# hmchuong/MaGGIe

Hardware: AMD Instinct MI355X
Metric: instance-frames/sec (fwd+bwd+optimizer step, 512x512, bf16) (higher is better)
Workload: dtype bf16

## Files before the change

include/maggie_hip.h:

```cpp
#ifndef MAGGIE_HIP_H
#define MAGGIE_HIP_H
#include <stdint.h>
#ifdef __cplusplus
extern "C" {
#endif

#define MG_F32 0
#define MG_BF16 1
#define MG_F16 3

#define MG_ACT_NONE 0
#define MG_ACT_RELU 1
#define MG_ACT_LRELU 2

#define MG_STAT_REPLICAS 32

#define MG_MODE_CONV 0
#define MG_MODE_TCONV 1
#define MG_MODE_GATHER 2

int mg_abi_version(void);
int mg_set_zeroed_range(void* base, long bytes);
int mg_zero_claim(void* p, long bytes);
int mg_zeroed_range_conflicts(void);

#define MG_DET_STAT_ROWS 1024
int mg_set_deterministic(int on);
int mg_get_deterministic(void);
int mg_det_init(long bytes);
int mg_det_side_stream(void* stream, long bytes);
int mg_stat_rows(void);
int mg_det_reduce_test(const float* slots, int nblk, int groups, int nv, float* dst, void* stream);

typedef struct mg_conv_params {
    const void* x;
    const void* w;
    void* y;
    const int32_t* nbr;
    const float* scale;
    const float* shift;
    const void* res;
    const void* res2;
    float* stats;
    int32_t dtype, mode;
    int32_t N, Hin, Win, Cin, Hout, Wout, Cout, R, S, stride, pad, dil;
    int32_t M;
    int32_t ldx, ldy, yoff, ldr, ldr2;
    int32_t act, pre_act, res_mode;
    float slope;
    int32_t dw_dtype;
    int32_t stat_mode;
    const int32_t* m_dev;
    const void* bnb_y;
    const void* bnb_x;
    const float* bnb_mean;
    const float* bnb_invstd;
    int32_t bnb_act, bnb_ld;
    int32_t stat_rep;
    int32_t reserved0;
    const float* xf_scale;
    const float* xf_shift;
    int32_t xf_act;
    float xf_slope;
    const float* bnb_scale;
    const float* bnb_shift;
} mg_conv_params;

int mg_conv_xform_ok(const mg_conv_params* p, int which);

int mg_conv_fprop(const mg_conv_params* p, void* stream);
int mg_set_halo3(int on);
int mg_set_halo3_cfg(int th, int bn, int ns);
int mg_conv_stat_rows(int M, int N, int Hout, int Wout);
int mg_coop_error(int* out);
int mg_set_bn_coop(int on);
int mg_set_bn_bwd_tail(int on);
long mg_conv_fprop_workspace(const mg_conv_params* p);
int mg_conv_fprop_ws(const mg_conv_params* p, float* workspace, long workspace_floats, void* stream);

int mg_conv_wgrad(const mg_conv_params* p, void* stream);
long mg_conv_wgrad_workspace(const mg_conv_params* p);
int mg_conv_wgrad_ws(const mg_conv_params* p, float* workspace, long workspace_floats, void* stream);
typedef struct mg_wgrad_parked {
    const float* ws;
    void* dw;
    long n;
    int32_t splits, form, dw_dtype, blocks;
} mg_wgrad_parked;
int mg_conv_wgrad_park(const mg_conv_params* p, float* workspace, long workspace_floats, mg_wgrad_parked* out, void* stream);
int mg_wgrad_reduce_batched(const mg_wgrad_parked* items, int count, void* stream);


typedef struct mg_rowwise_params {
    const void* x;
    void* y;
    const void* dy;
    void* dx;
    const void* res;
    const void* res2;
    void* dres;
    const float* scale;
    const float* shift;
    const float* mean;
    const float* invstd;
    float* sums;
    const float* count_ptr;
    int32_t dtype, M, C, H, W;
    int32_t ldx, ldy, yoff, ldr, ldr2, lddy, lddx, lddres;
    int32_t act, res_mode, mask_x_pos;
    float slope, count;
    const int32_t* m_dev;
    int32_t count_mult;
    int32_t mask_from_x;
} mg_rowwise_params;

int mg_colstats(const void* x, int dtype, int M, int C, int ld, float* stats, void* stream);
int mg_colstats_centered(const void* x, int dtype, int M, int C, int ld, float* stats, int have_sum, void* stream);
int mg_stat_rows_sum(const float* stats, int nrep, int n, float* out, void* stream);
int mg_bn_finalize(const float* stats, int nrep, const float* count_ptr, float count, int C, int centered, const float* gamma, const float* beta,
                   float* running_mean, float* running_var, float momentum, float eps, float* scale, float* shift,
                   float* mean_out, float* invstd_out, void* stream);
int mg_bn_train_fwd(const mg_rowwise_params* p, float* stats_ws, int ws_zeroed, float* outs, const float* stats_in, int stats_in_rows,
                    int exact, const float* gamma, const float* beta, float* running_mean, float* running_var, float momentum, float eps,
                    void* stream);
int mg_bn_train_bwd(const mg_rowwise_params* p, int sums_zeroed, void* stream);
int mg_bn_fold(int C, const float* gamma, const float* beta, const float* running_mean, const float* running_var,
               float eps, float* scale, float* shift, void* stream);
int mg_affine_act(const mg_rowwise_params* p, void* stream);
int mg_bn_bwd_reduce(const mg_rowwise_params* p, void* stream);
int mg_bn_bwd_apply(const mg_rowwise_params* p, void* stream);
int mg_bn_bwd_apply_linked(const mg_rowwise_params* p, const float* sums_rep, int nrep, float* sums_out, void* stream);
int mg_pool2x2(const void* in, void* out, int dtype, int op, int N, int Ho, int Wo, int C, void* stream);

#define MG_U8 2
int mg_bits_pack(const void* a, int dtype, void* bits, int P, int H, int W, int mode, float lo, float hi, void* stream);
int mg_bits_unpack_u8(const void* bits, uint8_t* out, int P, int H, int W, void* stream);
int mg_bits_unpack_f32(const void* bits, float* out, int P, int H, int W, void* stream);
int mg_bits_select(const void* bits, const float* a, const float* b, float* out, int P, int H, int W, void* stream);
int mg_bits_select_bwd(const void* bits, const float* dy, float* da, float* db, int P, int H, int W, void* stream);
int mg_bits_dilate(const void* in, void* out, const void* andmask, int P, int H, int W, const int32_t* widths, int width_all,
                   void* stream);
int mg_bits_downsample(const void* fine, void* coarse, int P, int Hf, int Wf, void* stream);
int mg_bits_rank(const void* bits, int P, int H, int W, int32_t* counts_tmp, int32_t* rowoff, int32_t* wordoff, void* stream);
int mg_bits_truncate(void* bits, const int32_t* wordoff, int P, int H, int W, int cap, int32_t* count, int32_t* overflow, void* stream);
int mg_bits_coords(const void* bits, const int32_t* wordoff, int P, int H, int W, int32_t* coords, void* stream);
int mg_gather_table(const int32_t* coords, int R, int ksize, int kind, const void* src_bits, const int32_t* src_wordoff, int Hs,
                    int Ws, int32_t* nbr, void* stream);

int mg_gather_rows(const void* dense, int dtype, const int32_t* coords, int R, int n_i, int Hd, int Wd, int C, const float* mul,
                   int mul_ninst, void* out, int ldo, int yoff, void* stream);
int mg_gather_rows_bwd(const void* dout, int dtype, int ldo, int yoff, const int32_t* coords, int R, int n_i, int Hd, int Wd, int C,
                       const float* mul, int mul_ninst, const void* dense, float* ddense, float* dmul, void* stream);
int mg_gather_rows_dmul_det(const void* dout, int dtype, int ldo, int yoff, const int32_t* coords, int R, int n_i, int N, int Hd, int Wd, int C,
                            int mul_ninst, const void* dense, float* dmul, const int32_t* r_dev, void* stream);
int mg_gather_rows_bwd_dense(const void* dout, int dtype, int ldo, int yoff, const void* bits, const int32_t* wordoff, int n_i, int N,
                             int Hd, int Wd, int C, const float* mul, int mul_ninst, void* ddense, void* stream);
int mg_scatter_plane(const void* vals, int dtype, int ldv, int col, const int32_t* coords, int R, int P, int H, int W, float fill,
                     float* plane, void* stream);
int mg_gather_plane(const float* plane, const int32_t* coords, int R, int H, int W, void* vals, int dtype, int ldv, int col,
                    void* stream);
int mg_mask_embed(const float* image, const float* masks, const float* table, int N, int H, int W, int n_m, int Hm, int Wm,
                  int n_embed, void* out, int dtype, void* stream);
int mg_mask_embed_bwd(const void* dx, int dtype, const float* masks, int N, int H, int W, int n_m, int Hm, int Wm, int n_embed,
                      float* dtable, void* stream);
int mg_upsample_tanh(const void* in, int dtype, long sn, long sc, long sy, long sx, int N, int C, int h, int w, int scale,
                     int apply_tanh, float* out, void* stream);
int mg_upsample_tanh_bwd(const float* dout, const float* out, long sn, long sc, long sy, long sx, int N, int C, int h, int w,
                         int scale, int apply_tanh, float* din, void* stream);
int mg_upsample_tanh_ex(const void* in, int dtype, long sn, long sc, long sy, long sx, int N, int C, int h, int w, int scale,
                        int apply_tanh, float* out, const float* pscale, int32_t* any_nonzero, void* stream);
int mg_upsample_tanh_bwd_ex(const float* dout, const float* out, long sn, long sc, long sy, long sx, int N, int C, int h, int w,
                            int scale, int apply_tanh, float* din, const float* pscale, void* stream);

int mg_spectral_norm(const float* W, float* u, float* v, int A, int B, int taps, int transposed, int pad_in, void* out,
                     int out_dtype, float* work, void* stream);
int mg_spectral_norm_bwd(const float* G, const float* W, const float* u, const float* v, int A, int B, int taps, int transposed,
                         int pad_in, float* work, float* dW, void* stream);

int mg_attn_tok_fwd(const float* qk, const float* btab, const float* feat, const int32_t* ids, int B, int T, int L, int D, int NID,
                    float scale, float* p, float* ctx, void* stream);
int mg_attn_tok_bwd(const float* p, const float* feat, const float* qk, const int32_t* ids, const float* dctx, const float* dp, int B, int T,
                    int L, int D, int NID, float scale, float* gbuf, float* rowdot, float* dqk, float* dbtab, float* dfeat, void* stream);
int mg_attn_feat_fwd(const float* feat, const float* kq, const float* b2, const float* vp, const float* obias, const uint8_t* pad_mask,
                     const int32_t* ids, int B, int T, int L, int D, int NID, float scale, float* out, float* p, void* stream);
int mg_attn_feat_bwd(const float* dout, const float* p, const float* feat, const float* kq, const float* vp, const int32_t* ids, int B, int T,
                     int L, int D, int NID, float scale, float* dfeat, float* dkq, float* dvp, float* db2, float* dobias, void* stream);
int mg_attn_feat_fwd_ex(const float* feat, const float* kq, const float* b2, const float* vp, const float* obias, const uint8_t* pad_mask,
                        const int32_t* ids, int B, int T, int L, int Dm, int NID, float scale, float* out, float* p, int b2_tn, void* stream);
int mg_attn_feat_bwd_ex(const float* dout, const float* p, const float* feat, const float* kq, const float* vp, const int32_t* ids, int B, int T,
                        int L, int Dm, int NID, float scale, float* dfeat, float* dkq, float* dvp, float* db2, float* dobias, int b2_tn, void* stream);

int mg_plane_flags(const float* w, int P, int HW, int32_t* flags, void* stream);
int mg_plane_flags_ex(const float* w, int P, int HW, void* flags, int as_float, void* stream);
int mg_os8_weight(const float* gt, const float* a8, int P, long HW, int reweight, int32_t* flags_scratch, float* out, void* stream);
int mg_os8_weight_ex(const float* gt, const float* a8, int P, long HW, int reweight, int32_t* flags_scratch, float* out, const int32_t* pvalid,
                     void* stream);
int mg_loss_finish(const float* sums, float* out3, void* stream);
int mg_loss_coef(const float* g3, const float* sums, float* coef5, void* stream);
int mg_loss_point_fwd(const float* p, const float* t, const float* w, const int32_t* flags, int P, int H, int W, float* d,
                      float* sums, const int32_t* pvalid, void* stream);
int mg_pyr_down(const float* x, const int32_t* flags, int P, int h, int w, float* out, void* stream);
int mg_pyr_lap_fwd(const float* x, const float* down, const float* w0, int lvl, int H0, int W0, const int32_t* flags, int P, int h,
                   int w, float* G, float* sums, void* stream);
int mg_pyr_upT(const float* q, const float* coef, const float* add, const int32_t* flags, int P, int h, int w, float* r, void* stream);
int mg_pyr_downT(const float* r, const float* q, const float* coef, const int32_t* flags, int P, int h, int w, float* dd, void* stream);
int mg_loss_point_bwd(const float* p, const float* t, const float* w, const int32_t* flags, int P, int H, int W, const float* coef_rec,
                      const float* coef_grad, const float* dd, float* A, float* B, float* dp, const int32_t* pvalid, void* stream);

int mg_matting_losses_fwd(const float* const* p, const float* t, const float* const* w, const int32_t* pvalid, int S, int P, int H, int W, int32_t* flags,
                          float* d, float* down0, float* down1, float* down2, float* G0, float* G1, float* G2, float* sums, float* out, void* stream);
int mg_matting_losses_bwd(const float* g, const float* sums, const float* const* p, const float* t, const float* const* w, const int32_t* pvalid,
                          const int32_t* flags, int S, int P, int H, int W, const float* G0, const float* G1, const float* G2, float* coef, float* r2,
                          float* dd2, float* r1, float* dd1, float* r0, float* dd0, float* A, float* B, float* dp, void* stream);

typedef struct mg_sn_desc {
    const float* W;
    float* u;
    float* v;
    int64_t out_off;
    int64_t work_off;
    int64_t dw_off;
    int32_t A, B, taps, transposed, pad_in;
    int32_t plain;
    int32_t k3_first, k3_count;
} mg_sn_desc;
// ... 153 lines not shown
```

maggie_amd/csrc/conv_wgrad.hip:

```cpp
#include "common.h"
#include "conv_xcd.h"
#include "../../include/maggie_hip.h"
#include <stdlib.h>
#include <type_traits>

#define MG_STAMP(i)

namespace {

typedef __attribute__((ext_vector_type(4))) short s16x4;
typedef s16x4 __attribute__((address_space(3))) * lds_s16x4_ptr;

template <typename T, int TCO, int TCI, int MODE, bool XF = false>
__global__ __launch_bounds__(256) void igemm_wgrad_kernel(const mg_conv_params p, int rows_per_block, float* __restrict__ ws) {
    using TR = ElemTraits<T>;
    constexpr int CE = TR::CE;
    constexpr bool BF = sizeof(T) == 2;
    constexpr int KSTEP = BF ? 128 : 64;
    constexpr int WROWS = KSTEP / 4;
    constexpr int PAD = BF ? 8 : 16;
    constexpr int PCO = TCO + PAD, PCI = TCI + PAD;
    constexpr int CPY = TCO / CE, CPX = TCI / CE;
    constexpr int ITY = (KSTEP * CPY) / 256, ITX = (KSTEP * CPX) / 256;
    constexpr int FM = TCO / 16, FN = TCI / 16;
    static_assert((KSTEP * CPY) % 256 == 0 && (KSTEP * CPX) % 256 == 0, "tile/threads mismatch");

    extern __shared__ __attribute__((aligned(16))) char smem[];
    T* sY = (T*)smem;
    T* sX = (T*)(smem + KSTEP * PCO * sizeof(T));

    const int t = threadIdx.x, lane = t & 63, wave = t >> 6;
    const int li = lane & 15, g = lane >> 4;
    const int taps = p.R * p.S;
    const int nci = (p.Cin + TCI - 1) / TCI;
    const int nco = (p.Cout + TCO - 1) / TCO;
    int nsplit = (p.M + rows_per_block - 1) / rows_per_block;
    const int M = dev_rows(p.m_dev, p.M);
    if (p.m_dev) {
        rows_per_block = (((M + nsplit - 1) / nsplit + KSTEP - 1) / KSTEP) * KSTEP;
        if (rows_per_block < KSTEP) rows_per_block = KSTEP;
    }
    int work;
    if (!xcd_order(nsplit * taps * nci * nco, work)) return;
    const int tc = work % (taps * nci);
    const int rest = work / (taps * nci);
    const int split = rest / nco;
    const int tap = tc / nci;
    const int ci0 = (tc - tap * nci) * TCI;
    const int co0 = (rest - split * nco) * TCO;
    const int mbeg = split * rows_per_block;
    const int mend = min(M, mbeg + rows_per_block);
    if (mbeg >= mend && !p.m_dev) return;
    const int ky = tap / p.S, kx = tap - ky * p.S;
    const FastDiv div_hw(MODE == MG_MODE_GATHER ? 1 : p.Hout * p.Wout), div_w(MODE == MG_MODE_GATHER ? 1 : p.Wout);
    const int sshift = p.stride == 1 ? 0 : (p.stride == 2 ? 1 : (p.stride == 4 ? 2 : -1));
    const T* __restrict__ yb = (const T*)p.y;
    const T* __restrict__ xb = (const T*)p.x;
    const bool yvec = (p.ldy % CE == 0) && (p.yoff % CE == 0);

    uint4 ry[ITY], rx[ITX];
    [[maybe_unused]] float xsc[CE < 8 ? 8 : CE], xsh[CE < 8 ? 8 : CE];
    [[maybe_unused]] unsigned xlive = 0;
    [[maybe_unused]] const float xsl = xf_slope_of(p.xf_act, p.xf_slope);
    if constexpr (XF) {
        static_assert(BF && 256 % CPX == 0, "operand transform: 16-bit storage, one channel group per thread");
        const int c = t % CPX;
#pragma unroll
        for (int e = 0; e < 8; ++e) {
            const int ci = ci0 + c * CE + e;
            xsc[e] = ci < p.Cin ? p.xf_scale[ci] : 0.f; xsh[e] = ci < p.Cin ? p.xf_shift[ci] : 0.f;
        }
    }
    auto load_step = [&](int mb) {
#pragma unroll
        for (int i = 0; i < ITY; ++i) {
            int idx = t + i * 256;
            int row = idx / CPY, c = idx - row * CPY;
            int m = mb + row, co = co0 + c * CE;
            uint4 q = make_uint4(0, 0, 0, 0);
            if (m < mend && co < p.Cout) {
                const T* src = yb + (long)m * p.ldy + p.yoff + co;
                if (yvec && co + CE <= p.Cout) q = *(const uint4*)src;
                else {
                    float f[CE];
#pragma unroll
                    for (int e = 0; e < CE; ++e) f[e] = (co + e < p.Cout) ? TR::ld(src + e) : 0.f;
                    q = TR::pack(f);
                }
            }
            ry[i] = q;
        }
#pragma unroll
        for (int i = 0; i < ITX; ++i) {
            int idx = t + i * 256;
            int row = idx / CPX, c = idx - row * CPX;
            int m = mb + row, ci = ci0 + c * CE;
            long src = -1;
            if (m < mend && ci < p.Cin) {
                if (MODE == MG_MODE_GATHER) {
                    src = p.nbr[(long)m * taps + tap];
                } else {
                    int n, rem, ho, wo;
                    div_hw.divmod(m, n, rem);
                    div_w.divmod(rem, ho, wo);
                    if (MODE == MG_MODE_CONV) {
                        int hi = ho * p.stride - p.pad + ky * p.dil, wi = wo * p.stride - p.pad + kx * p.dil;
                        if (hi >= 0 && hi < p.Hin && wi >= 0 && wi < p.Win) src = ((long)n * p.Hin + hi) * p.Win + wi;
                    } else {
                        int th = ho + p.pad - ky * p.dil, tw = wo + p.pad - kx * p.dil;
                        if (th >= 0 && tw >= 0) {
                            int hi, wi;
                            if (sshift >= 0) { hi = th >> sshift; wi = tw >> sshift; }
                            else { hi = th / p.stride; wi = tw / p.stride; }
                            if (hi * p.stride == th && wi * p.stride == tw && hi < p.Hin && wi < p.Win)
                                src = ((long)n * p.Hin + hi) * p.Win + wi;
                        }
                    }
                }
            }
            rx[i] = (src >= 0) ? *(const uint4*)(xb + src * p.ldx + ci) : make_uint4(0, 0, 0, 0);
            if constexpr (XF) xlive = src >= 0 ? (xlive | (1u << i)) : (xlive & ~(1u << i));
        }
    };
    auto store_step = [&]() {
#pragma unroll
        for (int i = 0; i < ITY; ++i) {
            int idx = t + i * 256; int row = idx / CPY, c = idx - row * CPY;
            *(uint4*)(sY + row * PCO + c * CE) = ry[i];
        }
#pragma unroll
        for (int i = 0; i < ITX; ++i) {
            int idx = t + i * 256; int row = idx / CPX, c = idx - row * CPX;
            if constexpr (XF) { if (xlive & (1u << i)) rx[i] = xf_apply8<T>(rx[i], xsc, xsh, xsl); }
            *(uint4*)(sX + row * PCI + c * CE) = rx[i];
        }
    };

    f32x4 acc[FM][FN];
#pragma unroll
    for (int i = 0; i < FM; ++i)
#pragma unroll
        for (int j = 0; j < FN; ++j) acc[i][j] = (f32x4){0.f, 0.f, 0.f, 0.f};

    const int wr = wave * WROWS;
    load_step(mbeg);
    for (int mb = mbeg; mb < mend; mb += KSTEP) {
        store_step();
        __syncthreads();
        if (mb + KSTEP < mend) load_step(mb + KSTEP);
        if constexpr (BF) {
            s16x4 a[FM][2], b[FN][2];
            const int r0 = wr + g * 4 + (li >> 2), cq = (li & 3) * 4;
#pragma unroll
            for (int i = 0; i < FM; ++i) {
                a[i][0] = __builtin_amdgcn_ds_read_tr16_b64_v4i16((lds_s16x4_ptr)(sY + r0 * PCO + i * 16 + cq));
                a[i][1] = __builtin_amdgcn_ds_read_tr16_b64_v4i16((lds_s16x4_ptr)(sY + (r0 + 16) * PCO + i * 16 + cq));
            }
#pragma unroll
            for (int j = 0; j < FN; ++j) {
// ... 495 lines not shown
    constexpr int ITY = NY / 256;
    extern __shared__ __attribute__((aligned(16))) char smem[];
    bf16raw* sY = (bf16raw*)smem;
    bf16raw* sX = sY + TH * TW * PY;

    const int t = threadIdx.x, lane = t & 63, wave = t >> 6;
    const int li = lane & 15, g = lane >> 4;
    const int mt = wave & 1, pair = wave >> 1;
    const int nco = p.Cout / TCO;
    const int tiles_x = (p.Wout + TW - 1) / TW, tiles_y = (p.Hout + TH - 1) / TH;
    const int S = p.N * tiles_y * tiles_x;
    const int nsplit = (S + tiles_per_block - 1) / tiles_per_block;
    int work;
    if (!xcd_order(nsplit * nco, work)) return;
    const int co0 = (work % nco) * TCO, split = work / nco;
    const int s_beg = split * tiles_per_block, s_end = min(S, s_beg + tiles_per_block);
    const bf16raw* __restrict__ yb = (const bf16raw*)p.y;
    const bf16raw* __restrict__ xb = (const bf16raw*)p.x;

    int y_ty[ITY], y_tx[ITY], y_off[ITY];
#pragma unroll
    for (int i = 0; i < ITY; ++i) {
        const int idx = t + i * 256;
        const int px = idx >> 2, c = idx & 3;
        y_ty[i] = px / TW; y_tx[i] = px % TW;
        y_off[i] = (y_ty[i] * p.Wout + y_tx[i]) * p.ldy + c * 8;
    }
    const int x_hy = t < NX ? t / HW_ - 1 : (1 << 20), x_hx = t % HW_ - 1;
    const int x_off = t < NX ? (x_hy * p.Win + x_hx) * p.ldx : 0;
    if (t < 4) *(uint4*)(sX + (NX + t) * 8) = make_uint4(0, 0, 0, 0);
    uint4 ry[ITY], rx;
    auto load_tile = [&](int s) {
        const int n = s / (tiles_y * tiles_x);
        const int r = s - n * tiles_y * tiles_x;
        const int y0 = (r / tiles_x) * TH, x0 = (r % tiles_x) * TW;
        const bf16raw* ybase = yb + ((long)(n * p.Hout + y0) * p.Wout + x0) * p.ldy + p.yoff + co0;
        const bf16raw* xbase = xb + ((long)(n * p.Hin + y0) * p.Win + x0) * p.ldx;
#pragma unroll
        for (int i = 0; i < ITY; ++i)
            ry[i] = (y0 + y_ty[i] < p.Hout && x0 + y_tx[i] < p.Wout) ? *(const uint4*)(ybase + y_off[i]) : make_uint4(0, 0, 0, 0);
        rx = ((unsigned)(y0 + x_hy) < (unsigned)p.Hin && (unsigned)(x0 + x_hx) < (unsigned)p.Win) ? *(const uint4*)(xbase + x_off) : make_uint4(0, 0, 0, 0);
    };
    auto store_tile = [&]() {
#pragma unroll
        for (int i = 0; i < ITY; ++i) {
            const int idx = t + i * 256;
            *(uint4*)(sY + (idx >> 2) * PY + (idx & 3) * 8) = ry[i];
        }
        if (t < NX) *(uint4*)(sX + t * 8) = rx;
    };

    f32x4 acc[3];
#pragma unroll
    for (int ky = 0; ky < 3; ++ky) acc[ky] = (f32x4){0.f, 0.f, 0.f, 0.f};
    const int q = g * 4 + (li >> 2), cq = (li & 3) * 4;
    if (s_beg < s_end) load_tile(s_beg);
    for (int s = s_beg; s < s_end; ++s) {
        store_tile();
        __syncthreads();
        if (s + 1 < s_end) load_tile(s + 1);
#pragma unroll
        for (int kc = 0; kc < TH / 2; ++kc) {
            union { s16x4 h[2]; uint4 v; } ua, ub;
            ua.h[0] = __builtin_amdgcn_ds_read_tr16_b64_v4i16((lds_s16x4_ptr)(sY + ((2 * kc) * TW + q) * PY + mt * 16 + cq));
            ua.h[1] = __builtin_amdgcn_ds_read_tr16_b64_v4i16((lds_s16x4_ptr)(sY + ((2 * kc + 1) * TW + q) * PY + mt * 16 + cq));
#pragma unroll
            for (int ky = 0; ky < 3; ++ky) {
                ub.h[0] = __builtin_amdgcn_ds_read_tr16_b64_v4i16((lds_s16x4_ptr)(sX + ((2 * kc + ky) * HW_ + q + 2 * pair) * 8 + cq));
                ub.h[1] = __builtin_amdgcn_ds_read_tr16_b64_v4i16((lds_s16x4_ptr)(sX + ((2 * kc + 1 + ky) * HW_ + q + 2 * pair) * 8 + cq));
                acc[ky] = mfma16<T>(ua.v, ub.v, acc[ky]);
            }
        }
        __syncthreads();
    }
    float* __restrict__ slab = ws + (long)split * p.Cout * 72;
    const int kx = 2 * pair + (li >> 3), ci = li & 7;
    if (kx < 3) {
#pragma unroll
        for (int ky = 0; ky < 3; ++ky)
#pragma unroll
            for (int e = 0; e < 4; ++e)
                slab[((long)(co0 + mt * 16 + g * 4 + e) * 9 + ky * 3 + kx) * 8 + ci] = acc[ky][e];
    }
}

static inline bool wgrad_c8_eligible(const mg_conv_params& p) {
    static const int on = [] { const char* e = getenv("MG_WGRAD_C8"); return e ? atoi(e) : 1; }();
    return on && MG_IS16(p.dtype) && p.mode == MG_MODE_CONV && !p.m_dev && p.R == 3 && p.S == 3 && p.stride == 1 && p.pad == 1 && p.dil == 1 &&
           p.Hout == p.Hin && p.Wout == p.Win && p.Cin == 8 && p.Cout % 32 == 0 && p.ldx % 8 == 0 && p.ldy % 8 == 0 && p.yoff % 8 == 0 &&
           p.Wout >= 16 && p.Hout >= 8;
}
static long plan_wgrad_c8(const mg_conv_params& p, int* tpb_out) {
    const long S = (long)p.N * ((p.Hout + 7) / 8) * ((p.Wout + 15) / 16);
    const long nco = p.Cout / 32;
    long splits = (512 + nco - 1) / nco;
    if (splits > S) splits = S;
    if (splits < 1) splits = 1;
    const int tpb = (int)((S + splits - 1) / splits);
    splits = (S + tpb - 1) / tpb;
    if (tpb_out) *tpb_out = tpb;
    return splits;
}
static int launch_wgrad_c8(const mg_conv_params& p, float* ws, long ws_floats, hipStream_t st) {
    int tpb = 1;
    const long splits = plan_wgrad_c8(p, &tpb);
    const long n = (long)p.Cout * 72;
    const bool out_bf16 = MG_IS16(p.dw_dtype);
    if (!ws || ws_floats < splits * n) return -4;
    dim3 grid(xcd_grid(splits * (p.Cout / 32)));
    const size_t lds = (size_t)(8 * 16 * (32 + 16) + (10 * 18 + 4) * 8) * sizeof(bf16raw);
    if (p.dtype == MG_F16) hipLaunchKernelGGL(igemm_wgrad_c8_kernel<f16raw>, grid, dim3(256), lds, st, p, tpb, ws);
    else hipLaunchKernelGGL(igemm_wgrad_c8_kernel<bf16raw>, grid, dim3(256), lds, st, p, tpb, ws);
    const long b = (n + 31) / 32;
    MG_REDUCE_LAUNCH(wgrad_reduce_tile_kernel, b, ws, splits);
    MG_CHECK_LAUNCH();
    return 0;
}

static inline bool wgrad_halo_eligible(const mg_conv_params& p) {
    static const int on = [] { const char* e = getenv("MG_WGRAD_HALO"); return e ? atoi(e) : 1; }();
    return on && MG_IS16(p.dtype) && p.mode == MG_MODE_CONV && !p.m_dev && p.R == 3 && p.S == 3 && p.stride == 1 && p.pad == 1 && p.dil == 1 &&
           p.Hout == p.Hin && p.Wout == p.Win && p.Cin % 32 == 0 && p.Cout % 32 == 0 && p.ldx % 8 == 0 && p.ldy % 8 == 0 && p.yoff % 8 == 0 &&
           p.Wout >= 16 && p.Hout >= 8 && (long)p.Cout * 9 * p.Cin <= (16l << 20);
}

struct WgradHaloPlan { long splits; int tpb; };

static WgradHaloPlan plan_wgrad_halo(const mg_conv_params& p) {
    const long cc = (long)(p.Cin / 32) * (p.Cout / 32);
    const long S = (long)p.N * ((p.Hout + 7) / 8) * ((p.Wout + 15) / 16);
    static const long target = [] { const char* e = getenv("MG_WGRAD_HALO_BLOCKS"); return e ? atol(e) : 256l; }();
    const long n = (long)p.Cout * 9 * p.Cin;
    long splits = (target + cc - 1) / cc;
    if (splits > S) splits = S;
    if (splits > (16l << 20) / n) splits = (16l << 20) / n;
    if (splits < 1) splits = 1;
    const int tpb = (int)((S + splits - 1) / splits);
    splits = (S + tpb - 1) / tpb;
    return {splits, tpb};
}

static int launch_wgrad_halo(const mg_conv_params& p, float* ws, long ws_floats, hipStream_t st) {
    const WgradHaloPlan pl = plan_wgrad_halo(p);
    const long n = (long)p.Cout * 9 * p.Cin;
    const bool out_bf16 = MG_IS16(p.dw_dtype);
    float* use_ws = nullptr;
    if ((pl.splits > 1 || out_bf16) && ws && ws_floats >= pl.splits * n) use_ws = ws;
    if (out_bf16 && !use_ws) return -4;
    if (pl.splits > 1 && !use_ws) return -4;
    if (pl.splits == 1 && !out_bf16) use_ws = p.stats;
    const long cc = (long)(p.Cin / 32) * (p.Cout / 32);
    dim3 grid(xcd_grid(pl.splits * cc));
    const size_t lds = (size_t)(8 * 16 * (32 + 16) + 10 * 18 * (32 + 16)) * sizeof(bf16raw);
    if (p.xf_scale) {
        if (p.dtype == MG_F16) hipLaunchKernelGGL((igemm_wgrad_halo_kernel<1, 1, f16raw, true>), grid, dim3(256), lds, st, p, pl.tpb, use_ws);
        else hipLaunchKernelGGL((igemm_wgrad_halo_kernel<1, 1, bf16raw, true>), grid, dim3(256), lds, st, p, pl.tpb, use_ws);
    } else if (p.dtype == MG_F16) hipLaunchKernelGGL((igemm_wgrad_halo_kernel<1, 1, f16raw>), grid, dim3(256), lds, st, p, pl.tpb, use_ws);
    else hipLaunchKernelGGL((igemm_wgrad_halo_kernel<1, 1>), grid, dim3(256), lds, st, p, pl.tpb, use_ws);
    if (use_ws != p.stats) {
        if (pl.splits >= 8) {
            const long b = (n + 31) / 32;
            MG_REDUCE_LAUNCH(wgrad_reduce_tile_kernel, b, use_ws, pl.splits);
        } else {
            long b = (n + 255) / 256; if (b > 2048) b = 2048;
            MG_REDUCE_LAUNCH(wgrad_reduce_kernel, b, use_ws, pl.splits);
        }
    }
    MG_CHECK_LAUNCH();
    return 0;
}

struct WgradPlan { long splits; int rpb; };

template <typename T, int TCO, int TCI>
WgradPlan plan_wgrad(const mg_conv_params& p) {
    constexpr int KSTEP = sizeof(T) == 2 ? 128 : 64;
    const int taps = p.R * p.S;
    const int nci = (p.Cin + TCI - 1) / TCI, nco = (p.Cout + TCO - 1) / TCO;
    const long tiles = (long)taps * nci * nco;
    static const long target = [] { const char* e = getenv("MG_WGRAD_BLOCKS"); return e ? atol(e) : 256l; }();
    const long n = (long)p.Cout * taps * p.Cin;
    long splits = p.M / (8 * KSTEP);
    static const long target_split = [] { const char* e = getenv("MG_WGRAD_BLOCKS_SPLIT"); return e ? atol(e) : 768l; }();
    long lo = ((splits > 1 ? target_split : target) + tiles - 1) / tiles;
    long by_rows = (p.M + 2 * KSTEP - 1) / (2 * KSTEP);
    if (lo > by_rows) lo = by_rows;
    if (splits < lo) splits = lo;
    if (splits > 2048 / tiles) splits = 2048 / tiles;
    if (splits > 512) splits = 512;
    if (splits > (16l << 20) / n) splits = (16l << 20) / n;
    if (p.m_dev) {
        static const long dev_splits = [] { const char* e = getenv("MG_WGRAD_DEV_SPLITS"); return e ? atol(e) : 128l; }();
        const long cap = (dev_splits * 9 + tiles - 1) / tiles;
        if (splits > cap) splits = cap;
    }
    if (splits < 1) splits = 1;
    int rpb = (int)((p.M + splits - 1) / splits);
    rpb = ((rpb + KSTEP - 1) / KSTEP) * KSTEP;
    splits = (p.M + rpb - 1) / rpb;
    return {splits, rpb};
}

template <typename T, int TCO, int TCI>
int launch_wgrad(const mg_conv_params& p, float* ws, long ws_floats, hipStream_t st) {
    constexpr bool BF = sizeof(T) == 2;
    constexpr int KSTEP = BF ? 128 : 64;
    constexpr int PAD = BF ? 8 : 16;
    const int taps = p.R * p.S;
    const int nci = (p.Cin + TCI - 1) / TCI, nco = (p.Cout + TCO - 1) / TCO;
    WgradPlan pl = plan_wgrad<T, TCO, TCI>(p);
    const long n = (long)p.Cout * taps * p.Cin;
    const bool out_bf16 = MG_IS16(p.dw_dtype);
    float* use_ws = nullptr;
    if ((pl.splits > 1 || out_bf16) && ws && ws_floats >= pl.splits * n) use_ws = ws;
    if (out_bf16 && !use_ws) return -4;
    mg_conv_params q = p;
    if (pl.splits == 1 && !out_bf16) use_ws = p.stats;
    dim3 grid(xcd_grid((long)pl.splits * taps * nci * nco));
    size_t stage = (size_t)KSTEP * (TCO + PAD + TCI + PAD) * sizeof(T);
    size_t red = (size_t)4 * TCO * (TCI + 1) * 4;
    size_t lds = stage > red ? stage : red;
    if (p.xf_scale) {
        if constexpr (BF && TCO == 32 && TCI == 32) {
            if (p.mode == MG_MODE_CONV) hipLaunchKernelGGL((igemm_wgrad_kernel<T, TCO, TCI, MG_MODE_CONV, true>), grid, dim3(256), lds, st, q, pl.rpb, use_ws);
            else if (p.mode == MG_MODE_GATHER) hipLaunchKernelGGL((igemm_wgrad_kernel<T, TCO, TCI, MG_MODE_GATHER, true>), grid, dim3(256), lds, st, q, pl.rpb, use_ws);
            else return MG_XF_UNSUPPORTED;
        } else return MG_XF_UNSUPPORTED;
    } else
    switch (p.mode) {
        case MG_MODE_CONV: hipLaunchKernelGGL((igemm_wgrad_kernel<T, TCO, TCI, MG_MODE_CONV>), grid, dim3(256), lds, st, q, pl.rpb, use_ws); break;
        case MG_MODE_TCONV: hipLaunchKernelGGL((igemm_wgrad_kernel<T, TCO, TCI, MG_MODE_TCONV>), grid, dim3(256), lds, st, q, pl.rpb, use_ws); break;
        case MG_MODE_GATHER: hipLaunchKernelGGL((igemm_wgrad_kernel<T, TCO, TCI, MG_MODE_GATHER>), grid, dim3(256), lds, st, q, pl.rpb, use_ws); break;
        default: return -2;
    }
    if (use_ws && (pl.splits > 1 || out_bf16)) {
        if (pl.splits > 32 && n <= (1l << 16)) {
            long b = (n + 3) / 4; if (b > 8192) b = 8192;
            MG_REDUCE_LAUNCH(wgrad_reduce_wave_kernel, b, use_ws, pl.splits);
        } else {
            long b = (n + 255) / 256; if (b > 2048) b = 2048;
            MG_REDUCE_LAUNCH(wgrad_reduce_kernel, b, use_ws, pl.splits);
        }
    }
    MG_CHECK_LAUNCH();
    return 0;
}

static inline bool wgrad_xf_rows_ok(const mg_conv_params& p) {
    if (!MG_IS16(p.dtype) || !p.m_dev || p.Cout > 32 || p.ldx % 8) return false;
    if (p.mode == MG_MODE_GATHER && p.R * p.S == 9) return p.Cin == 32 || (p.Cin == 64 && wgrad_gather9_eligible(p));
    return p.mode == MG_MODE_CONV && p.R * p.S == 1 && p.stride == 1 && p.pad == 0 && p.Cin == 32;
}
static inline bool wgrad_xf_ok(const mg_conv_params& p) {
    return (MG_IS16(p.dtype) && wgrad_halo_eligible(p) && !wgrad_c8_eligible(p) && !wgrad_gather9_eligible(p)) || wgrad_xf_rows_ok(p);
}

template <typename T>
int dispatch_wgrad(const mg_conv_params& p, float* ws, long ws_floats, long* need, hipStream_t st) {
    const bool small_co = p.Cout <= 32, small_ci = p.Cin <= 32;
    const long n = (long)p.Cout * p.R * p.S * p.Cin;
    if (p.xf_scale && !wgrad_xf_ok(p)) { if (need) { *need = 0; return 0; } return MG_XF_UNSUPPORTED; }
    if (sizeof(T) == 2 && wgrad_c8_eligible(p)) {
        const long splits = plan_wgrad_c8(p, nullptr);
        if (need) { *need = splits * n; return 0; }
        if (ws && ws_floats >= splits * n) return launch_wgrad_c8(p, ws, ws_floats, st);
    }
    if (sizeof(T) == 2 && wgrad_gather9_eligible(p)) {
        const long splits = plan_wgrad_gather9(p);
        if (need) { *need = splits * n; return 0; }
        if (ws && ws_floats >= splits * n) return launch_wgrad_gather9(p, ws, ws_floats, st);
    }
    if (sizeof(T) == 2 && wgrad_halo_eligible(p)) {
        if (need) { const WgradHaloPlan pl = plan_wgrad_halo(p); *need = (pl.splits > 1 || MG_IS16(p.dw_dtype)) ? pl.splits * n : 0; return 0; }
        const WgradHaloPlan pl = plan_wgrad_halo(p);
        if (pl.splits == 1 || (ws && ws_floats >= pl.splits * n)) return launch_wgrad_halo(p, ws, ws_floats, st);
    }
    if (p.xf_scale && !wgrad_xf_rows_ok(p)) return MG_XF_UNSUPPORTED;
#define MG_WG(TCO, TCI)                                                                             \
    do {                                                                                            \
        if (need) { WgradPlan pl = plan_wgrad<T, TCO, TCI>(p); *need = (pl.splits > 1 || MG_IS16(p.dw_dtype)) ? pl.splits * n : 0; return 0; } \
        return launch_wgrad<T, TCO, TCI>(p, ws, ws_floats, st);                                     \
    } while (0)
    if (small_co && small_ci) MG_WG(32, 32);
    if (small_co) MG_WG(32, 64);
    if (small_ci) MG_WG(64, 32);
    MG_WG(64, 64);
#undef MG_WG
}

int wgrad_check(const mg_conv_params* pp) {
    if (!pp) return -1;
    const mg_conv_params& p = *pp;
    const int ce = MG_IS16(p.dtype) ? 8 : 4;
    if (p.Cin % ce != 0 || p.ldx % ce != 0) return -3;
    if (p.mode == MG_MODE_GATHER && !p.nbr) return -5;
    if (!MG_IS16(p.dtype) && p.dtype != MG_F32) return -6;
    if (MG_IS16(p.dw_dtype) && p.dw_dtype != p.dtype) return -6;
    return 0;
}

}

bool mg_wgrad_xform_ok(const mg_conv_params& p) { return wgrad_xf_ok(p); }

extern "C" long mg_conv_wgrad_workspace(const mg_conv_params* pp) {
    if (wgrad_check(pp) || pp->M <= 0) return 0;
    long need = 0;
    if (MG_IS16(pp->dtype)) dispatch_wgrad<bf16raw>(*pp, nullptr, 0, &need, nullptr);
    else dispatch_wgrad<float>(*pp, nullptr, 0, &need, nullptr);
    return need;
}
// ... 57 lines not shown
```

Baseline: 767.8.

## Add warp-specialized pipelined wgrad halo kernel with async global-to-LDS loads

Adds a new 3x3 weight-gradient kernel that splits each 512-thread block into producer waves, which stream dy and halo'd x tiles into a multi-stage LDS ring using global_load_lds, and consumer waves, which run MFMA on transposed LDS reads. It is enabled by default through an environment toggle and falls back to the old halo kernel if the LDS attribute cannot be set. The aim is to hide global-load latency behind MFMA work and drop register staging. In exchange it uses more LDS per block, relies on hand-tuned vmcnt waits, and assumes the tile shape matches the existing split plan.

```diff
diff --git a/include/maggie_hip.h b/include/maggie_hip.h
--- a/include/maggie_hip.h
+++ b/include/maggie_hip.h
@@ -71,6 +71,7 @@
 int mg_conv_fprop(const mg_conv_params* p, void* stream);
 int mg_set_halo3(int on);
 int mg_set_halo3_cfg(int th, int bn, int ns);
+int mg_set_wgrad_h3(int on);
 int mg_conv_stat_rows(int M, int N, int Hout, int Wout);
 int mg_coop_error(int* out);
 int mg_set_bn_coop(int on);
diff --git a/maggie_amd/csrc/conv_wgrad.hip b/maggie_amd/csrc/conv_wgrad.hip
--- a/maggie_amd/csrc/conv_wgrad.hip
+++ b/maggie_amd/csrc/conv_wgrad.hip
@@ -5,6 +5,9 @@
 #include <type_traits>
 
 #define MG_STAMP(i)
+
+bool mg_wgrad_h3_on();
+int mg_wgrad_h3_gemm(const mg_conv_params& p, int tiles_per_block, long splits, float* slabs, hipStream_t st);
 
 namespace {
 
@@ -806,11 +809,15 @@
     const long cc = (long)(p.Cin / 32) * (p.Cout / 32);
     dim3 grid(xcd_grid(pl.splits * cc));
     const size_t lds = (size_t)(8 * 16 * (32 + 16) + 10 * 18 * (32 + 16)) * sizeof(bf16raw);
-    if (p.xf_scale) {
-        if (p.dtype == MG_F16) hipLaunchKernelGGL((igemm_wgrad_halo_kernel<1, 1, f16raw, true>), grid, dim3(256), lds, st, p, pl.tpb, use_ws);
-        else hipLaunchKernelGGL((igemm_wgrad_halo_kernel<1, 1, bf16raw, true>), grid, dim3(256), lds, st, p, pl.tpb, use_ws);
-    } else if (p.dtype == MG_F16) hipLaunchKernelGGL((igemm_wgrad_halo_kernel<1, 1, f16raw>), grid, dim3(256), lds, st, p, pl.tpb, use_ws);
-    else hipLaunchKernelGGL((igemm_wgrad_halo_kernel<1, 1>), grid, dim3(256), lds, st, p, pl.tpb, use_ws);
+    const int h3 = mg_wgrad_h3_on() ? mg_wgrad_h3_gemm(p, pl.tpb, pl.splits, use_ws, st) : 1;
+    if (h3 < 0) return h3;
+    if (h3 == 1) {
+        if (p.xf_scale) {
+            if (p.dtype == MG_F16) hipLaunchKernelGGL((igemm_wgrad_halo_kernel<1, 1, f16raw, true>), grid, dim3(256), lds, st, p, pl.tpb, use_ws);
+            else hipLaunchKernelGGL((igemm_wgrad_halo_kernel<1, 1, bf16raw, true>), grid, dim3(256), lds, st, p, pl.tpb, use_ws);
+        } else if (p.dtype == MG_F16) hipLaunchKernelGGL((igemm_wgrad_halo_kernel<1, 1, f16raw>), grid, dim3(256), lds, st, p, pl.tpb, use_ws);
+        else hipLaunchKernelGGL((igemm_wgrad_halo_kernel<1, 1>), grid, dim3(256), lds, st, p, pl.tpb, use_ws);
+    }
     if (use_ws != p.stats) {
         if (pl.splits >= 8) {
             const long b = (n + 31) / 32;
diff --git a/maggie_amd/csrc/conv_wgrad_h3.hip b/maggie_amd/csrc/conv_wgrad_h3.hip
--- /dev/null
+++ b/maggie_amd/csrc/conv_wgrad_h3.hip
@@ -0,0 +1,228 @@
+#include "common.h"
+#include "conv_xcd.h"
+#include "../../include/maggie_hip.h"
+#include <stdlib.h>
+
+namespace {
+
+__device__ uint4 mg_wh3_zero_page[4];
+
+typedef __attribute__((ext_vector_type(4))) short s16x4;
+typedef s16x4 __attribute__((address_space(3))) * lds_s16x4_ptr;
+typedef __attribute__((ext_vector_type(4))) unsigned int u32x4;
+typedef __attribute__((address_space(3))) void* lds_void_ptr;
+typedef const __attribute__((address_space(1))) void* gbl_void_ptr;
+
+template <int NS_> struct WH3 {
+    static constexpr int TH = 8, TW = 16, HH = TH + 2, PW = 24, NS = NS_;
+    static constexpr int Y_BYTES = TH * TW * 64;
+    static constexpr int X_PIECES = (HH * PW + 15) / 16;
+    static constexpr int X_PER_WAVE = (X_PIECES + 3) / 4;
+    static constexpr int Y_PER_WAVE = TH * TW / 16 / 4;
+    static constexpr int L = X_PER_WAVE + Y_PER_WAVE;
+    static constexpr int STAGE = Y_BYTES + X_PER_WAVE * 4 * 1024;
+    static constexpr int LDS = NS * STAGE;
+    static_assert(NS >= 2 && (NS - 1) * L <= 63, "vmcnt is a 6-bit counter");
+};
+
+template <int N> __device__ __forceinline__ void wh3_wait_vm() { asm volatile("s_waitcnt vmcnt(%0)" ::"n"(N) : "memory"); }
+template <int J, int L> __device__ __forceinline__ void wh3_wait_stages(int infl) {
+    if constexpr (J <= 0) wh3_wait_vm<0>();
+    else if (infl >= J) wh3_wait_vm<J * L>();
+    else wh3_wait_stages<J - 1, L>(infl);
+}
+
+template <typename T, bool XF, int NS>
+__global__ __launch_bounds__(512) void wgrad_h3_kernel(const mg_conv_params p, int tiles_per_block, float* __restrict__ ws) {
+    using C = WH3<NS>;
+    constexpr int TH = C::TH, TW = C::TW, PW = C::PW;
+    constexpr int Y_BYTES = C::Y_BYTES, STAGE = C::STAGE, L = C::L, XPW = C::X_PER_WAVE, YPW = C::Y_PER_WAVE;
+    constexpr int TCO = 32, TCI = 32;
+    extern __shared__ __attribute__((aligned(16))) char smem[];
+
+    const int t = threadIdx.x, lane = t & 63, wave = (t >> 6) & 3;
+    const bool producer = (t >> 8) != 0;
+    const int nci = p.Cin / TCI, nco = p.Cout / TCO;
+    const int tiles_x = (p.Wout + TW - 1) / TW, tiles_y = (p.Hout + TH - 1) / TH;
+    const int S = p.N * tiles_y * tiles_x;
+    const int nsplit = (S + tiles_per_block - 1) / tiles_per_block;
+    int work;
+    if (!xcd_order(nsplit * nco * nci, work)) return;
+    const int cc = work % (nco * nci), split = work / (nco * nci);
+    const int co0 = (cc / nci) * TCO, ci0 = (cc % nci) * TCI;
+    const int s_beg = split * tiles_per_block, s_end = min(S, s_beg + tiles_per_block);
+    const int nst = s_end - s_beg;
+    const int H = p.Hout, W = p.Wout;
+
+    if (producer) {
+        const int ch = (lane & 3) ^ (((lane >> 4) & 1) * 2);
+        int x_hy[XPW], x_hx[XPW];
+#pragma unroll
+        for (int i = 0; i < XPW; ++i) {
+            const int q = (wave + 4 * i) * 16 + (lane >> 2);
+            x_hy[i] = q / PW; x_hx[i] = q - (q / PW) * PW;
+            if (wave + 4 * i >= C::X_PIECES || x_hx[i] >= TW + 2) x_hy[i] = -(1 << 20);
+        }
+        const char* __restrict__ xb = (const char*)p.x + (long)ci0 * 2 + ch * 16;
+        const char* __restrict__ yb = (const char*)p.y + (long)(p.yoff + co0) * 2 + ch * 16;
+        const char* zpage = (const char*)mg_wh3_zero_page;
+        const long xpitch = (long)p.ldx * 2, ypitch = (long)p.ldy * 2;
+        [[maybe_unused]] float xsc[8], xsh[8];
+        [[maybe_unused]] const float xsl = xf_slope_of(p.xf_act, p.xf_slope);
+        if constexpr (XF) {
+#pragma unroll
+            for (int e = 0; e < 8; ++e) { xsc[e] = p.xf_scale[ci0 + ch * 8 + e]; xsh[e] = p.xf_shift[ci0 + ch * 8 + e]; }
+        }
+        auto origin = [&](int s, int& n, int& y0, int& x0) {
+            n = s / (tiles_y * tiles_x);
+            const int r = s - n * tiles_y * tiles_x;
+            y0 = (r / tiles_x) * TH; x0 = (r % tiles_x) * TW;
+        };
+        auto x_in = [&](int i, int y0, int x0) {
+            return (unsigned)(y0 - 1 + x_hy[i]) < (unsigned)H && (unsigned)(x0 - 1 + x_hx[i]) < (unsigned)W;
+        };
+        auto issue_stage = [&](int s, int buf) {
+            int n, y0, x0;
+            origin(s, n, y0, x0);
+            char* sbase = smem + buf * STAGE;
+#pragma unroll
+            for (int i = 0; i < YPW; ++i) {
+                const int ty = wave + 4 * i, tx = lane >> 2;
+                const bool ok = y0 + ty < H && x0 + tx < W;
+                const char* g = ok ? yb + ((long)(n * H + y0 + ty) * W + x0 + tx) * ypitch : zpage;
+                __builtin_amdgcn_global_load_lds((gbl_void_ptr)g, (lds_void_ptr)(sbase + (wave + 4 * i) * 1024), 16, 0, 0);
+            }
+#pragma unroll
+            for (int i = 0; i < XPW; ++i) {
+                const char* g = x_in(i, y0, x0) ? xb + ((long)(n * H + y0 - 1 + x_hy[i]) * W + x0 - 1 + x_hx[i]) * xpitch : zpage;
+                __builtin_amdgcn_global_load_lds((gbl_void_ptr)g, (lds_void_ptr)(sbase + Y_BYTES + (wave + 4 * i) * 1024), 16, 0, 0);
+            }
+        };
+        [[maybe_unused]] auto xf_stage = [&](int s, int buf) {
+            int n, y0, x0;
+            origin(s, n, y0, x0);
+            const unsigned sb = (unsigned)(size_t)(__attribute__((address_space(3))) char*)smem + (unsigned)(buf * STAGE + Y_BYTES);
+            u32x4 q[XPW];
+#pragma unroll
+            for (int i = 0; i < XPW; ++i)
+                asm volatile("ds_read_b128 %0, %1" : "=v"(q[i]) : "v"(sb + (unsigned)((wave + 4 * i) * 1024 + lane * 16)) : "memory");
+            asm volatile("s_waitcnt lgkmcnt(0)" ::: "memory");
+#pragma unroll
+            for (int i = 0; i < XPW; ++i) {
+                const u32x4 w_ = x_in(i, y0, x0) ? __builtin_bit_cast(u32x4, xf_apply8<T>(__builtin_bit_cast(uint4, q[i]), xsc, xsh, xsl)) : q[i];
+                asm volatile("ds_write_b128 %0, %1" ::"v"(sb + (unsigned)((wave + 4 * i) * 1024 + lane * 16)), "v"(w_) : "memory");
+            }
+            asm volatile("s_waitcnt lgkmcnt(0)" ::: "memory");
+        };
+        issue_stage(s_beg, 0);
+        wh3_wait_vm<0>();
+        if constexpr (XF) xf_stage(s_beg, 0);
+        __builtin_amdgcn_s_barrier();
+#pragma unroll
+        for (int u = 1; u < NS; ++u)
+            if (u < nst) issue_stage(s_beg + u, u);
+        int fbuf = 0;
+        for (int k = 1; k < nst; ++k) {
+            wh3_wait_stages<NS - 2, L>(min(NS - 1, nst - k) - 1);
+            const int buf = fbuf + 1 == NS ? 0 : fbuf + 1;
+            if constexpr (XF) xf_stage(s_beg + k, buf);
+            __builtin_amdgcn_s_barrier();
+            if (k + NS - 1 < nst) issue_stage(s_beg + k + NS - 1, fbuf);
+            fbuf = buf;
+        }
+        return;
+    }
+
+    const int li = lane & 15, g = lane >> 4;
+    const int wco = (wave >> 1) * 16, wci = (wave & 1) * 16;
+    const int q = g * 4 + (li >> 2), cq = (li & 3) * 4;
+    const unsigned y_lane = (unsigned)(q * 64 + ((((wco + cq) >> 3) ^ ((g & 1) * 2)) << 4) + (cq & 7) * 2);
+    unsigned x_lane[3];
+#pragma unroll
+    for (int kx = 0; kx < 3; ++kx) {
+        const int col = q + kx;
+        x_lane[kx] = (unsigned)(Y_BYTES + col * 64 + ((((wci + cq) >> 3) ^ (((col >> 2) & 1) * 2)) << 4) + (cq & 7) * 2);
+    }
+    f32x4 acc[9];
+#pragma unroll
+    for (int tp = 0; tp < 9; ++tp) acc[tp] = (f32x4){0.f, 0.f, 0.f, 0.f};
+
+    int buf = 0;
+    for (int k = 0; k < nst; ++k) {
+        asm volatile("s_waitcnt lgkmcnt(0)" ::: "memory");
+        __builtin_amdgcn_s_barrier();
+        asm volatile("" ::: "memory");
+        char* sb = smem + buf * STAGE;
+        buf = buf + 1 == NS ? 0 : buf + 1;
+#pragma unroll
+        for (int kc = 0; kc < TH / 2; ++kc) {
+            union { s16x4 h[2]; uint4 v; } ua;
+            ua.h[0] = __builtin_amdgcn_ds_read_tr16_b64_v4i16((lds_s16x4_ptr)(sb + y_lane + (2 * kc) * TW * 64));
+            ua.h[1] = __builtin_amdgcn_ds_read_tr16_b64_v4i16((lds_s16x4_ptr)(sb + y_lane + (2 * kc + 1) * TW * 64));
+#pragma unroll
+            for (int ky = 0; ky < 3; ++ky)
+#pragma unroll
+                for (int kx = 0; kx < 3; ++kx) {
+                    union { s16x4 h[2]; uint4 v; } ub;
+                    ub.h[0] = __builtin_amdgcn_ds_read_tr16_b64_v4i16((lds_s16x4_ptr)(sb + x_lane[kx] + (2 * kc + ky) * PW * 64));
+                    ub.h[1] = __builtin_amdgcn_ds_read_tr16_b64_v4i16((lds_s16x4_ptr)(sb + x_lane[kx] + (2 * kc + 1 + ky) * PW * 64));
+                    acc[ky * 3 + kx] = mfma16<T>(ua.v, ub.v, acc[ky * 3 + kx]);
+                }
+        }
+    }
+    float* __restrict__ slab = ws + (long)split * p.Cout * 9 * p.Cin;
+#pragma unroll
+    for (int tp = 0; tp < 9; ++tp)
+#pragma unroll
+        for (int e = 0; e < 4; ++e)
+            slab[((long)(co0 + wco + g * 4 + e) * 9 + tp) * p.Cin + ci0 + wci + li] = acc[tp][e];
+}
+
+constexpr int WH3_MAX_DEVICES = 16;
+constexpr int WH3_NS = 3;
+int g_wh3_attr[WH3_MAX_DEVICES] = {};
+
+template <int NS>
+hipError_t wh3_attr() {
+    constexpr int lds = WH3<NS>::LDS;
+    hipError_t e = hipFuncSetAttribute((const void*)wgrad_h3_kernel<bf16raw, false, NS>, hipFuncAttributeMaxDynamicSharedMemorySize, lds);
+    if (e == hipSuccess) e = hipFuncSetAttribute((const void*)wgrad_h3_kernel<bf16raw, true, NS>, hipFuncAttributeMaxDynamicSharedMemorySize, lds);
+    if (e == hipSuccess) e = hipFuncSetAttribute((const void*)wgrad_h3_kernel<f16raw, false, NS>, hipFuncAttributeMaxDynamicSharedMemorySize, lds);
+    if (e == hipSuccess) e = hipFuncSetAttribute((const void*)wgrad_h3_kernel<f16raw, true, NS>, hipFuncAttributeMaxDynamicSharedMemorySize, lds);
+    return e;
+}
+
+template <int NS>
+int wh3_launch(const mg_conv_params& p, int tiles_per_block, long splits, float* slabs, hipStream_t st, int dev) {
+    if (g_wh3_attr[dev] == 0) g_wh3_attr[dev] = wh3_attr<NS>() == hipSuccess ? 1 : -1;
+    if (g_wh3_attr[dev] < 0) return 1;
+    const long cc = (long)(p.Cin / 32) * (p.Cout / 32);
+    const dim3 grid(xcd_grid(splits * cc));
+    const size_t lds = WH3<NS>::LDS;
+    if (p.xf_scale) {
+        if (p.dtype == MG_F16) hipLaunchKernelGGL((wgrad_h3_kernel<f16raw, true, NS>), grid, dim3(512), lds, st, p, tiles_per_block, slabs);
+        else hipLaunchKernelGGL((wgrad_h3_kernel<bf16raw, true, NS>), grid, dim3(512), lds, st, p, tiles_per_block, slabs);
+    } else if (p.dtype == MG_F16) hipLaunchKernelGGL((wgrad_h3_kernel<f16raw, false, NS>), grid, dim3(512), lds, st, p, tiles_per_block, slabs);
+    else hipLaunchKernelGGL((wgrad_h3_kernel<bf16raw, false, NS>), grid, dim3(512), lds, st, p, tiles_per_block, slabs);
+    const hipError_t e = hipGetLastError();
+    return e == hipSuccess ? 0 : -(int)e;
+}
+
+}
+
+static int g_wh3_on = -1;
+bool mg_wgrad_h3_on() {
+    if (g_wh3_on < 0) { const char* e = getenv("MG_WGRAD_H3"); g_wh3_on = e ? (atoi(e) != 0) : 1; }
+    return g_wh3_on != 0;
+}
+extern "C" int mg_set_wgrad_h3(int on) {
+    const int was = mg_wgrad_h3_on() ? 1 : 0;
+    g_wh3_on = on != 0;
+    return was;
+}
+
+int mg_wgrad_h3_gemm(const mg_conv_params& p, int tiles_per_block, long splits, float* slabs, hipStream_t st) {
+    int dev = 0;
+    if (hipGetDevice(&dev) != hipSuccess || dev < 0 || dev >= WH3_MAX_DEVICES) return 1;
+    return wh3_launch<WH3_NS>(p, tiles_per_block, splits, slabs, st, dev);
+}
```

Result: no change. 765.6, median of 3 (-0.3%).
